# ArmastusChen/Learning-Continuous-Implicit-Representation-for-Near-Periodic-Patterns

Measured on AMD Instinct MI355X. Metric: fitted pixels/sec/GPU (512^2 grid, 256-wide MLP) + iters-to-target-PSNR, higher is better.
Workload: dtype bf16

## Files before the change

### learning-continuous-implicit-representation-for-near-periodic-patterns_amd/csrc/npp_api.hip

```cpp
#include <math.h>
#include <stdarg.h>
#include <stdio.h>
#include <string.h>
#include <vector>

#include "npp_common.h"
#include "npp_stash_census.h"

namespace npp {

static thread_local char g_err[512] = "";

void set_error(const char* fmt, ...) {
  va_list ap;
  va_start(ap, fmt);
  vsnprintf(g_err, sizeof(g_err), fmt, ap);
  va_end(ap);
}

int check_launch(const char* what) {
  hipError_t e = hipGetLastError();
  if (e != hipSuccess) {
    set_error("%s: %s", what, hipGetErrorString(e));
    return NPP_ERR_LAUNCH;
  }
  return NPP_OK;
}

bool smem_attr(SmemOnce& once, const void* fn, int bytes) {
  int dev = 0;
  if (hipGetDevice(&dev) != hipSuccess) return false;
  const unsigned long long bit = 1ull << (dev & 63);
  if (__atomic_load_n(&once.done, __ATOMIC_RELAXED) & bit) return true;
  if (hipFuncSetAttribute(fn, hipFuncAttributeMaxDynamicSharedMemorySize, bytes) != hipSuccess) return false;
  __atomic_fetch_or(&once.done, bit, __ATOMIC_RELAXED);
  return true;
}

static const char* kNames[kNumLayers] = {
    "periodic_linears.0", "periodic_linears.1", "periodic_linears.2", "periodic_linears.3",
    "periodic_linears.4", "periodic_linears.5", "periodic_linears.6", "periodic_linears.7",
    "feature_linear1",    "scale_linears.0",    "feature_linear2",    "pos_linears.0",
    "rgb_linear"};
static char g_name_buf[kNumLayers * 2][40];

NPP_HD float fwd_pack_value(const float* P, const NetDesc& d, int l, int ks, int nt, int lane, int j) {
  const int col = fwd_col(d.K, l, ks, lane >> 5, j);
  if (col < 0) return 0.0f;
  const int row = nt * 32 + (lane & 31);
  return P[d.w_off[l] + (int64_t)row * d.n_in[l] + col];
}
NPP_HD float bwd_pack_value(const float* P, const NetDesc& d, const BwdDesc& b, int v, int ns, int kt,
                            int lane, int j) {
  const int l = b.layer[v];
  const int n = 16 * ns + perm16(lane >> 5, j);
  const int col = b.col0[v] + kt * 32 + (lane & 31);
  return P[d.w_off[l] + (int64_t)n * d.n_in[l] + col];
}

NPP_HD bool fwd_unit(const NetDesc& d, int64_t u, int& l, int& ks, int& nt, int& lane) {
  for (l = 0; l < kNumLayers; ++l) {
    if (!d.present[l] || d.nt_f[l] == 0) continue;
    const int64_t n = (int64_t)d.ks_f[l] * d.nt_f[l] * 64;
    if (u >= d.wf_off[l] && u < d.wf_off[l] + n) {
      int64_t r = u - d.wf_off[l];
      lane = (int)(r & 63);
      r >>= 6;
      nt = (int)(r % d.nt_f[l]);
      ks = (int)(r / d.nt_f[l]);
      return true;
    }
  }
  return false;
}
NPP_HD bool bwd_unit(const BwdDesc& b, int64_t u, int& v, int& ns, int& kt, int& lane) {
  for (v = 0; v < kNumBwd; ++v) {
    if (!b.present[v]) continue;
    const int64_t n = (int64_t)b.ns[v] * kNT * 64;
    if (u >= b.off16[v] && u < b.off16[v] + n) {
      int64_t r = u - b.off16[v];
      lane = (int)(r & 63);
      r >>= 6;
      kt = (int)(r % kNT);
      ns = (int)(r / kNT);
      return true;
    }
  }
  return false;
}

__global__ void pack_weights_kernel(const float* __restrict__ P, bf16x8* __restrict__ wf,
                                    bf16x8* __restrict__ wb, NetDesc d, BwdDesc b, int64_t nf,
                                    int64_t nb) {
  const int64_t u = (int64_t)blockIdx.x * blockDim.x + threadIdx.x;
  if (u < nf) {
    int l, ks, nt, lane;
    if (fwd_unit(d, u, l, ks, nt, lane)) {
      bf16x8 r;
#pragma unroll
      for (int j = 0; j < 8; ++j) r[j] = (__bf16)fwd_pack_value(P, d, l, ks, nt, lane, j);
      wf[u] = r;
    }
  } else if (u < nf + nb) {
    const int64_t ub = u - nf;
    int v, ns, kt, lane;
    if (bwd_unit(b, ub, v, ns, kt, lane)) {
      bf16x8 r;
#pragma unroll
      for (int j = 0; j < 8; ++j) r[j] = (__bf16)bwd_pack_value(P, d, b, v, ns, kt, lane, j);
      wb[ub] = r;
    }
  }
}

struct AdamPackArgs {
  float *p, *m, *v;
  const float* g;
  int64_t n;
  int32_t n_slabs;
  int64_t slab_stride;
  float step_size, b1, b2, inv_sqrt_bc2, eps;
  AdamTail tail;
  __bf16 *wf, *wb;
  uint32_t magic[kNumLayers];
  const StackIter* iter;
  int64_t blob_stride, slab_img_stride, wf_stride, wb_stride;
  int32_t lat_stride, zero_stride;
  int64_t pl_stride;
  const float* hp;
};

__global__ __launch_bounds__(256) void adam_pack_kernel(AdamPackArgs a_in, NetDesc d_arg, BwdDesc b_arg) {
  AdamPackArgs a = a_in;
  if (a.iter) {
    const int y = (int)blockIdx.y;
    const StackIter it = a.iter[y];
    if (!it.active) return;
    a.p += y * a.blob_stride; a.m += y * a.blob_stride; a.v += y * a.blob_stride;
    a.g += y * a.slab_img_stride;
    a.wf += y * a.wf_stride; a.wb += y * a.wb_stride;
    a.step_size = it.step_size; a.inv_sqrt_bc2 = it.inv_sqrt_bc2;
    a.tail.p += y * a.lat_stride; a.tail.m += y * a.lat_stride; a.tail.v += y * a.lat_stride; a.tail.g += y * a.lat_stride;
    a.tail.zero += y * a.zero_stride;
    if (a.tail.pl_part) a.tail.pl_part += y * a.pl_stride;
    if (a.tail.loss_cur) a.tail.loss_cur += y * a.zero_stride;
  }
  if (a.hp) { a.step_size = a.hp[0]; a.inv_sqrt_bc2 = a.hp[1]; }
  __shared__ NetDesc d;
  __shared__ BwdDesc b;
  __shared__ uint32_t magic[kNumLayers];
  if (threadIdx.x == 0) {
    const uint32_t* s1 = (const uint32_t*)&d_arg;
    uint32_t* t1 = (uint32_t*)&d;
#pragma unroll
    for (int i = 0; i < (int)(sizeof(NetDesc) / 4); ++i) t1[i] = s1[i];
    const uint32_t* s2 = (const uint32_t*)&b_arg;
    uint32_t* t2 = (uint32_t*)&b;
#pragma unroll
    for (int i = 0; i < (int)(sizeof(BwdDesc) / 4); ++i) t2[i] = s2[i];
#pragma unroll
    for (int i = 0; i < kNumLayers; ++i) magic[i] = a.magic[i];
  }
  __syncthreads();
  if ((int64_t)blockIdx.x * blockDim.x * 4 >= a.n) {
    adam_tail_block(a.tail, a.step_size, a.b1, a.b2, a.inv_sqrt_bc2, a.eps);
    return;
  }
  const int64_t i = ((int64_t)blockIdx.x * blockDim.x + threadIdx.x) * 4;
  if (i >= a.n) return;
  const int cnt = (int)(a.n - i < 4 ? a.n - i : 4);
  float pn[4];
  adam_quad(a.p, a.m, a.v, a.g, i, cnt, a.n_slabs, a.slab_stride, a.step_size, a.b1, a.b2, a.inv_sqrt_bc2, a.eps, pn);
  int l = 0;
#pragma unroll
  for (int q = 1; q < kNumLayers; ++q)
    if (d.present[q] && i >= d.w_off[q]) l = q;
  int64_t r = i - d.w_off[l];
  int n = (int)__umulhi((uint32_t)r, magic[l]), k = (int)r - n * d.n_in[l];
  bool fwd4 = false;
  if (cnt == 4 && n < d.n_out[l] && (k & 3) == 0 && k + 3 < d.n_in[l]) {
    const int64_t p0 = fwd_pack_pos(d, l, n, k), p3 = fwd_pack_pos(d, l, n, k + 3);
    if (p0 >= 0 && p3 == p0 + 3 && (p0 & 3) == 0) {
      typedef __bf16 bf16x4_t __attribute__((ext_vector_type(4)));
      const bf16x4_t w4 = {(__bf16)pn[0], (__bf16)pn[1], (__bf16)pn[2], (__bf16)pn[3]};
      *(bf16x4_t*)(a.wf + p0) = w4;
      fwd4 = true;
    }
  }
#pragma unroll
  for (int e = 0; e < 4; ++e) {
    if (e < cnt) {
      if (n < d.n_out[l]) {
        const __bf16 w = (__bf16)pn[e];
        if (!fwd4) {
          const int64_t pf = fwd_pack_pos(d, l, n, k);
          if (pf >= 0) a.wf[pf] = w;
        }
        const int64_t pb = bwd_pack_pos(b, l, n, k);
        if (pb >= 0) a.wb[pb] = w;
      }
      if (++k == d.n_in[l]) { k = 0; ++n; }
      if (n >= d.n_out[l] && i + e + 1 >= d.b_off[l] + d.n_out[l]) {
        do { ++l; } while (l < kNumLayers && !d.present[l]);
        if (l >= kNumLayers) break;
        n = 0; k = 0;
      }
    }
  }
}

static uint16_t f32_to_bf16_host(float f) {
  uint32_t u;
  memcpy(&u, &f, 4);
  if ((u & 0x7fffffffu) > 0x7f800000u) return (uint16_t)((u >> 16) | 0x40);
  u += 0x7FFF + ((u >> 16) & 1);
  return (uint16_t)(u >> 16);
}

__global__ void selftest_kernel(float* out) {
  const int lane = threadIdx.x & 63;
  const int m = lane & 31, h = lane >> 5;
  bf16x8 a, b;
#pragma unroll
  for (int j = 0; j < 8; ++j) {
    const int k = 8 * h + j;
    a[j] = (__bf16)(float)(((m * 3 + k * 5) % 5) - 2);
    b[j] = (__bf16)(float)(((k * 7 + m * 2) % 4) - 1);
  }
  f32x16 acc = {};
  acc = mfma_bf16(a, b, acc);
#pragma unroll
  for (int r = 0; r < 16; ++r) out[acc_row(r, h) * 32 + m] = acc[r];
  f32x16 y = {};
#pragma unroll
  for (int s = 0; s < 2; ++s) {
    bf16x8 x = pack_acc(acc, s), a2;
#pragma unroll
    for (int j = 0; j < 8; ++j) {
      const int k = 16 * s + perm16(h, j);
      a2[j] = (__bf16)(float)(((m * 5 + k * 3) % 7) - 3);
    }
    y = mfma_bf16(a2, x, y);
  }
#pragma unroll
  for (int r = 0; r < 16; ++r) out[1024 + acc_row(r, h) * 32 + m] = y[r];

  __shared__ __attribute__((aligned(16))) char tile[16384];
  for (int u = lane; u < 1024; u += 64) {
    const int hh = u & 1, b = (u >> 1) & 31, bt = (u >> 6) & 1, ks = u >> 7;
    bf16x8 f;
#pragma unroll
    for (int j = 0; j < 8; ++j) {
      const int feat = 16 * ks + perm16(hh, j), row = bt * 32 + b;
      f[j] = (__bf16)(float)(((7 * feat + 3 * row) % 251) - 125);
    }
    *(bf16x8*)(tile + wfmt_unit(8, 0, ks, bt, b, hh)) = f;
  }
  __syncthreads();
  for (int tt = 0; tt < 4; ++tt)
    for (int t = 0; t < 4; ++t) {
      const bf16x8 f = wfrag_read(tile, wfrag_offset(tt, t, lane));
#pragma unroll
      for (int j = 0; j < 8; ++j) out[2048 + ((tt * 4 + t) * 64 + lane) * 8 + j] = (float)f[j];
    }
}

static int tune_env(const char* name, int dflt) {
  const char* e = getenv(name);
  return e && *e ? atoi(e) : dflt;
}
Tunables g_tune = {tune_env("NPP_CONV_WINK", 1), tune_env("NPP_CONV_WIN", 1), tune_env("NPP_CONV_WSTAT", 1), tune_env("NPP_CONV_PAIR", 15),
                   tune_env("NPP_LIGHT_DET", 1), tune_env("NPP_STASH8", 1)};

}

using namespace npp;

extern "C" {

int npp_version(void) { return 100; }

int npp_tune(const char* key, int value) {
  struct { const char* k; int* v; } tab[] = {{"conv_wink", &g_tune.conv_wink}, {"conv_win", &g_tune.conv_win},
                                             {"conv_wstat", &g_tune.conv_wstat}, {"conv_pair", &g_tune.conv_pair},
                                             {"stash8", &g_tune.stash8}, {"light_det", &g_tune.light_det}};
  if (key)
    for (auto& t : tab)
      if (!strcmp(key, t.k)) {
        const int old = __atomic_load_n(t.v, __ATOMIC_RELAXED);
        if (value >= 0) __atomic_store_n(t.v, value, __ATOMIC_RELAXED);
        return old;
      }
  set_error("npp_tune: unknown key '%s'", key ? key : "(null)");
  return NPP_ERR_ARG;
}
const char* npp_last_error_string(void) { return g_err; }

int npp_device_count(void) {
  int n = 0;
  hipError_t e = hipGetDeviceCount(&n);
  if (e != hipSuccess) {
    set_error("hipGetDeviceCount: %s", hipGetErrorString(e));
    (void)hipGetLastError();
    return 0;
  }
  return n;
}

static int check_kw(int K, int width) {
  if (K < 1 || K > NPP_MAX_K) { set_error("K=%d outside [1,%d]", K, NPP_MAX_K); return NPP_ERR_ARG; }
  if (width != NPP_WIDTH) {
    set_error("width=%d: this build is specialised for width %d", width, NPP_WIDTH);
    return NPP_ERR_UNSUPPORTED;
  }
  return NPP_OK;
}

int npp_param_layout(int K, int width, const char** names, int64_t* offsets, int32_t* rows,
                     int32_t* cols, int64_t* total) {
  int rc = check_kw(K, width);
  if (rc) return rc;
  const NetDesc d = make_desc(K);
  int n = 0;
  for (int l = 0; l < kNumLayers; ++l) {
    if (!d.present[l]) continue;
    for (int wb = 0; wb < 2; ++wb) {
      snprintf(g_name_buf[n], sizeof(g_name_buf[n]), "%s.%s", kNames[l], wb ? "bias" : "weight");
      if (names) names[n] = g_name_buf[n];
      if (offsets) offsets[n] = wb ? d.b_off[l] : d.w_off[l];
      if (rows) rows[n] = d.n_out[l];
      if (cols) cols[n] = wb ? 1 : d.n_in[l];
      ++n;
    }
  }
  if (total) *total = d.total_params;
  return n;
}

int64_t npp_pack_bytes(int K, int width, int which) {
  if (check_kw(K, width)) return -1;
  return 16 * (which == 0 ? make_desc(K).wf_total16 : bwd_total16(K));
}

int npp_pack_weights(const float* d_params, void* d_wf, void* d_wb, int K, int width, void* stream) {
  int rc = check_kw(K, width);
  if (rc) return rc;
  if (!d_params || !d_wf || !d_wb) { set_error("npp_pack_weights: null pointer"); return NPP_ERR_ARG; }
  const NetDesc d = make_desc(K);
  const BwdDesc b = make_bwd_desc(K);
  const int64_t nf = d.wf_total16, nb = bwd_total16(K);
  const int threads = 256;
  const int64_t blocks = (nf + nb + threads - 1) / threads;
  hipLaunchKernelGGL(pack_weights_kernel, dim3((unsigned)blocks), dim3(threads), 0, (hipStream_t)stream,
                     d_params, (bf16x8*)d_wf, (bf16x8*)d_wb, d, b, nf, nb);
  return check_launch("npp_pack_weights");
}

int npp_pack_weights_host(const float* params, void* wf, void* wb, int K, int width) {
  int rc = check_kw(K, width);
  if (rc) return rc;
  const NetDesc d = make_desc(K);
  const BwdDesc b = make_bwd_desc(K);
  uint16_t* f = (uint16_t*)wf;
  uint16_t* g = (uint16_t*)wb;
  for (int64_t u = 0; u < d.wf_total16; ++u) {
    int l, ks, nt, lane;
    if (!fwd_unit(d, u, l, ks, nt, lane)) { set_error("fwd unit %lld unmapped", (long long)u); return NPP_ERR_ARG; }
    for (int j = 0; j < 8; ++j) f[u * 8 + j] = f32_to_bf16_host(fwd_pack_value(params, d, l, ks, nt, lane, j));
  }
  const int64_t nb = bwd_total16(K);
  for (int64_t u = 0; u < nb; ++u) {
    int v, ns, kt, lane;
    if (!bwd_unit(b, u, v, ns, kt, lane)) { set_error("bwd unit %lld unmapped", (long long)u); return NPP_ERR_ARG; }
    for (int j = 0; j < 8; ++j) g[u * 8 + j] = f32_to_bf16_host(bwd_pack_value(params, d, b, v, ns, kt, lane, j));
  }
  return NPP_OK;
}

int npp_pack_scatter_host(const float* params, void* wf, void* wb, int K, int width) {
  int rc = check_kw(K, width);
  if (rc) return rc;
  const NetDesc d = make_desc(K);
  const BwdDesc b = make_bwd_desc(K);
  uint16_t* f = (uint16_t*)wf;
  uint16_t* g = (uint16_t*)wb;
  memset(f, 0, (size_t)d.wf_total16 * 16);
  memset(g, 0, (size_t)bwd_total16(K) * 16);
  for (int l = 0; l < kNumLayers; ++l) {
    if (!d.present[l]) continue;
    for (int n = 0; n < d.n_out[l]; ++n)
      for (int k = 0; k < d.n_in[l]; ++k) {
        const uint16_t w = f32_to_bf16_host(params[d.w_off[l] + (int64_t)n * d.n_in[l] + k]);
        const int64_t pf = fwd_pack_pos(d, l, n, k), pb = bwd_pack_pos(b, l, n, k);
        if (pf >= 0) {
          if (pf >= d.wf_total16 * 8) { set_error("fwd_pack_pos out of range (l=%d n=%d k=%d)", l, n, k); return NPP_ERR_ARG; }
          f[pf] = w;
        }
        if (pb >= 0) {
          if (pb >= bwd_total16(K) * 8) { set_error("bwd_pack_pos out of range (l=%d n=%d k=%d)", l, n, k); return NPP_ERR_ARG; }
          g[pb] = w;
        }
      }
  }
  return NPP_OK;
}

static int adam_pack_go(AdamPackArgs a, float* d_p, float* d_m, float* d_v, const float* d_gslabs, int64_t n, int n_slabs,
                        int64_t slab_stride, const AdamTail& tail, float beta1, float beta2, float eps, int M, int K,
                        void* d_wf, void* d_wb, void* stream, const char* who, const char* need) {
  const NetDesc d = make_desc(K);
  if (n != d.total_params || !d_p || !d_m || !d_v || !d_gslabs || !d_wf || !d_wb || n_slabs < 1 || tail.n < 0 || tail.n_zero < 0 ||
      (tail.n > 0 && (!tail.p || !tail.m || !tail.v || !tail.g)) || (tail.n_zero > 0 && !tail.zero) || slab_stride % 4 ||
      (((uintptr_t)d_p | (uintptr_t)d_m | (uintptr_t)d_v | (uintptr_t)d_gslabs) & 15)) {
    set_error("%s: bad arguments (n=%lld, expected %lld parameters; %s)", who, (long long)n, (long long)d.total_params, need);
    return NPP_ERR_ARG;
  }
  a.p = d_p; a.m = d_m; a.v = d_v; a.g = d_gslabs; a.n = n; a.n_slabs = n_slabs; a.slab_stride = slab_stride;
  a.b1 = beta1; a.b2 = beta2; a.eps = eps;
  a.tail = tail;
  a.wf = (__bf16*)d_wf; a.wb = (__bf16*)d_wb;
  for (int l = 0; l < kNumLayers; ++l) a.magic[l] = d.present[l] ? (uint32_t)((1ull << 32) / (uint64_t)d.n_in[l]) + 1u : 0u;
  const int64_t threads = (n + 3) / 4;
  hipLaunchKernelGGL(adam_pack_kernel, dim3((unsigned)((threads + 255) / 256 + 1), (unsigned)M), dim3(256), 0, (hipStream_t)stream, a, d,
                     make_bwd_desc(K));
  return check_launch(who);
}
static int adam_pack_bad(const char* who, const char* what) {
  set_error("%s: bad arguments (%s)", who, what);
  return NPP_ERR_ARG;
}
static const char* const kAdamPackNeed = "16-byte aligned blobs, slab stride % 4 == 0";

int npp_adam_step_net_pack(float* d_p, float* d_m, float* d_v, const float* d_gslabs, int64_t n, int n_slabs,
                           int64_t slab_stride, float* d_lat, float* d_lat_m, float* d_lat_v, float* d_dlat, int n_lat,
                           float* d_zero, int n_zero, float lr, float beta1, float beta2, float eps, int step, int K,
                           int width, void* d_wf, void* d_wb, float* d_pl_partials, float* d_loss_cur, void* stream) {
  int rc = check_kw(K, width);
  if (rc) return rc;
  if (step < 1) return adam_pack_bad("npp_adam_step_net_pack", "step < 1");
  const AdamWords w = adam_words(lr, beta1, beta2, step);
  AdamPackArgs a{};
  a.step_size = w.step_size; a.inv_sqrt_bc2 = w.inv_sqrt_bc2;
  return adam_pack_go(a, d_p, d_m, d_v, d_gslabs, n, n_slabs, slab_stride,
                      AdamTail{d_lat, d_lat_m, d_lat_v, d_dlat, n_lat, d_zero, n_zero, d_pl_partials, d_loss_cur}, beta1, beta2, eps,
                      1, K, d_wf, d_wb, stream, "npp_adam_step_net_pack", kAdamPackNeed);
}

int npp_adam_step_net_pack_dev(float* d_p, float* d_m, float* d_v, const float* d_gslabs, int64_t n, int n_slabs,
                               int64_t slab_stride, float* d_lat, float* d_lat_m, float* d_lat_v, float* d_dlat, int n_lat,
                               float* d_zero, int n_zero, float beta1, float beta2, float eps, const float* d_hp, int K,
                               int width, void* d_wf, void* d_wb, float* d_pl_partials, float* d_loss_cur, void* stream) {
  int rc = check_kw(K, width);
  if (rc) return rc;
  if (!d_hp || ((uintptr_t)d_hp & 3)) return adam_pack_bad("npp_adam_step_net_pack_dev", "the device words: null or not 4-byte aligned");
  AdamPackArgs a{};
  a.hp = d_hp;
  return adam_pack_go(a, d_p, d_m, d_v, d_gslabs, n, n_slabs, slab_stride,
                      AdamTail{d_lat, d_lat_m, d_lat_v, d_dlat, n_lat, d_zero, n_zero, d_pl_partials, d_loss_cur}, beta1, beta2, eps,
                      1, K, d_wf, d_wb, stream, "npp_adam_step_net_pack_dev", kAdamPackNeed);
}

int npp_adam_step_net_pack_stack(float* d_p, float* d_m, float* d_v, int64_t blob_stride, const float* d_gslabs, int64_t n,
                                 int n_slabs, int64_t slab_stride, int64_t slab_img_stride, float* d_lat, float* d_lat_m,
                                 float* d_lat_v, float* d_dlat, int n_lat, int lat_stride, float* d_zero, int n_zero,
                                 int zero_stride, float beta1, float beta2, float eps, int M, int K, int width, void* d_wf,
                                 int64_t wf_stride_bytes, void* d_wb, int64_t wb_stride_bytes, float* d_pl_partials,
                                 int64_t pl_stride, float* d_loss_cur, const void* d_iter, void* stream) {
  int rc = check_kw(K, width);
  if (rc) return rc;
  if (!d_iter || M < 1 || M > NPP_MAX_STACK || blob_stride % 4 || slab_img_stride % 4 || blob_stride < n || wf_stride_bytes % 16 ||
      wb_stride_bytes % 16)
    return adam_pack_bad("npp_adam_step_net_pack_stack", "M, the iteration records or the per-image strides");
  AdamPackArgs a{};
  a.iter = (const StackIter*)d_iter;
  a.blob_stride = blob_stride; a.slab_img_stride = slab_img_stride; a.wf_stride = wf_stride_bytes / 2; a.wb_stride = wb_stride_bytes / 2;
  a.lat_stride = lat_stride; a.zero_stride = zero_stride; a.pl_stride = pl_stride;
  return adam_pack_go(a, d_p, d_m, d_v, d_gslabs, n, n_slabs, slab_stride,
                      AdamTail{d_lat, d_lat_m, d_lat_v, d_dlat, n_lat, d_zero, n_zero, d_pl_partials, d_loss_cur}, beta1, beta2, eps,
                      M, K, d_wf, d_wb, stream, "npp_adam_step_net_pack_stack", "16-byte aligned blobs and strides");
}

int npp_train_workspace(int K, int width, int64_t Bp, int ksplit, int64_t sizes[4]) {
  int rc = check_kw(K, width);
  if (rc) return rc;
  if (Bp <= 0 || Bp % kRowTile || ksplit < 1 || !sizes) { set_error("npp_train_workspace: bad Bp/ksplit"); return NPP_ERR_ARG; }
  sizes[0] = 0;
  sizes[1] = (int64_t)act_total_ks(K) * (Bp / kRowTile) * (2048 + 1024);
  sizes[2] = (int64_t)kDzTotalKs * (Bp / kRowTile) * 2048;
  sizes[3] = (int64_t)ksplit * slab_stride_of(make_desc(K).total_params) * 4;
  return NPP_OK;
}

int64_t npp_stash8_census_words(int K, int width) {
  if (check_kw(K, width)) return -1;
  return census_words(K);
}

int npp_stash8_census_layout(int K, int width, const char** names, int32_t* formats, int32_t* features, int64_t* offsets,
                             int64_t* tile_offset) {
  int rc = check_kw(K, width);
  if (rc) return rc;
  static thread_local char name_buf[kCensusMaxArrays][12];
  const CensusDesc d = make_census_desc(K, name_buf);
  for (int i = 0; i < d.n; ++i) {
    if (names) names[i] = name_buf[i];
    if (formats) formats[i] = d.a[i].side;
    if (features) features[i] = d.a[i].features;
    if (offsets) offsets[i] = (int64_t)i * kCensusEntry;
  }
  if (tile_offset) *tile_offset = (int64_t)d.n * kCensusEntry;
  return d.n;
}

static int census_check(const char* who, const void* actF, const void* dzF, int64_t Bp, int64_t n_rows, int K, int width, const void* rec) {
  int rc = check_kw(K, width);
  if (rc) return rc;
  if (!actF || !dzF || !rec || (((uintptr_t)actF | (uintptr_t)dzF) & 15) || ((uintptr_t)rec & 7)) {
    set_error("%s: null or misaligned pointer (stash arrays 16-byte, record 8-byte aligned)", who);
    return NPP_ERR_ARG;
  }
  if (Bp <= 0 || Bp % kRowTile || Bp / kRowTile > 65536 || n_rows < 1 || n_rows > Bp) {
    set_error("%s: bad Bp=%lld (a multiple of %d, <= %d rows) / n_rows=%lld (1..Bp)", who, (long long)Bp, kRowTile, 65536 * kRowTile, (long long)n_rows);
    return NPP_ERR_ARG;
  }
  return NPP_OK;
}

int npp_stash8_census(const void* d_actF, const void* d_dzF, int64_t Bp, int64_t n_rows, int K, int width, int64_t* d_record,
                      void* stream) {
  int rc = census_check("npp_stash8_census", d_actF, d_dzF, Bp, n_rows, K, width, d_record);
  if (rc) return rc;
  CensusArgs A{};
  A.n_wg = Bp / kRowTile; A.n_rows = n_rows;
  A.act8 = (const uint8_t*)d_actF + act8_region_base(K, A.n_wg);
  A.dz8 = (const uint8_t*)d_dzF;
  A.rec = (unsigned long long*)d_record;
  A.d = make_census_desc(K);
  hipStream_t s = (hipStream_t)stream;
  const int64_t words = (int64_t)A.d.n * kCensusEntry + NPP_CENSUS_TILE_WORDS;
  hipError_t e = hipMemsetAsync(d_record, 0, (size_t)words * 8, s);
  if (e == hipSuccess) e = hipMemsetAsync(d_record + (int64_t)A.d.n * kCensusEntry + NPP_CENSUS_SCALE_MIN, 0x7f, 8, s);
  if (e != hipSuccess) { set_error("npp_stash8_census: hipMemsetAsync: %s", hipGetErrorString(e)); return NPP_ERR_LAUNCH; }
  int max_nks = 0;
  for (int i = 0; i < A.d.n; ++i) max_nks = A.d.a[i].nks > max_nks ? A.d.a[i].nks : max_nks;
  const int64_t want = ((int64_t)max_nks * A.n_wg * 64 + 4 * kCensusThreads - 1) / (4 * kCensusThreads);
  const unsigned gx = (unsigned)(want < 1 ? 1 : (want > 64 ? 64 : want));
  hipLaunchKernelGGL(stash8_census_kernel, dim3(gx, (unsigned)A.d.n + 1), dim3(kCensusThreads), 0, s, A);
  return check_launch("npp_stash8_census");
}

int npp_stash8_census_host(const void* actF, const void* dzF, int64_t Bp, int64_t n_rows, int K, int width, int64_t* record) {
  int rc = census_check("npp_stash8_census_host", actF, dzF, Bp, n_rows, K, width, record);
  if (rc) return rc;
  const int64_t n_wg = Bp / kRowTile;
  stash8_census_host((const uint8_t*)actF + act8_region_base(K, n_wg), (const uint8_t*)dzF, n_wg, n_rows, K, record);
  return NPP_OK;
}

int npp_selftest_mfma(void* d_scratch, void* stream) {
  if (!d_scratch) { set_error("npp_selftest_mfma: null scratch"); return NPP_ERR_ARG; }
  hipStream_t s = (hipStream_t)stream;
  hipLaunchKernelGGL(selftest_kernel, dim3(1), dim3(64), 0, s, (float*)d_scratch);
  int rc = check_launch("npp_selftest_mfma");
  if (rc) return rc;
  std::vector<float> out(2048 + 8192);
  hipError_t e = hipMemcpyAsync(out.data(), d_scratch, (2048 + 8192) * sizeof(float), hipMemcpyDeviceToHost, s);
  if (e == hipSuccess) e = hipStreamSynchronize(s);
  if (e != hipSuccess) { set_error("selftest copy: %s", hipGetErrorString(e)); return NPP_ERR_LAUNCH; }
  int A[32][16], B[16][32], D[32][32], A2[32][32];
  for (int m = 0; m < 32; ++m)
    for (int k = 0; k < 16; ++k) { A[m][k] = ((m * 3 + k * 5) % 5) - 2; B[k][m] = ((k * 7 + m * 2) % 4) - 1; }
  for (int m = 0; m < 32; ++m)
    for (int k = 0; k < 32; ++k) A2[m][k] = ((m * 5 + k * 3) % 7) - 3;
  for (int i = 0; i < 32; ++i)
    for (int j = 0; j < 32; ++j) {
      int acc = 0;
      for (int k = 0; k < 16; ++k) acc += A[i][k] * B[k][j];
      D[i][j] = acc;
    }
  for (int i = 0; i < 32; ++i)
    for (int j = 0; j < 32; ++j) {
      if (out[i * 32 + j] != (float)D[i][j]) {
        set_error("selftest: plain MFMA lane map mismatch at (%d,%d): got %g want %d", i, j, out[i * 32 + j], D[i][j]);
        return NPP_ERR_SELFTEST;
      }
      int acc = 0;
      for (int k = 0; k < 32; ++k) acc += A2[i][k] * D[k][j];
      if (out[1024 + i * 32 + j] != (float)acc) {
        set_error("selftest: accumulator-as-operand chain mismatch at (%d,%d): got %g want %d", i, j,
                  out[1024 + i * 32 + j], acc);
        return NPP_ERR_SELFTEST;
      }
    }
  for (int tt = 0; tt < 4; ++tt)
    for (int t = 0; t < 4; ++t)
      for (int lane = 0; lane < 64; ++lane)
        for (int j = 0; j < 8; ++j) {
          const int feat = 32 * tt + (lane & 31), row = 16 * t + 8 * (lane >> 5) + j;
          const float want = (float)(((7 * feat + 3 * row) % 251) - 125);
          const float got = out[2048 + ((tt * 4 + t) * 64 + lane) * 8 + j];
          if (got != want) {
            set_error("selftest: W-format transposed read mismatch tt=%d t=%d lane=%d j=%d: got %g want %g", tt, t, lane, j, got, want);
            return NPP_ERR_SELFTEST;
          }
        }
  return NPP_OK;
}

}
```

Measured before the change: 46.99 million.

## Tile Adam pack kernel into 4x4 weight tiles with shuffle-transposed backward stores

Adam parameter updates for aligned weight layers are now assigned per 4x4 tile, with a host-side region table mapping blocks to layers. Each thread updates four contiguous weights, writes them vectorized to the forward pack, and exchanges values with three lanes via xor-shuffles so that it can store a transposed 4-wide vector into the backward pack. Previously those backward writes were scattered scalar stores. The shared descriptor copy is spread across all threads, and tail blocks exit before it. The cost is a larger kernel argument and more index math per thread.

New measurement: 46.84 million. No clear change (-0.3%).

```diff
diff --git a/learning-continuous-implicit-representation-for-near-periodic-patterns_amd/csrc/npp_api.hip b/learning-continuous-implicit-representation-for-near-periodic-patterns_amd/csrc/npp_api.hip
--- a/learning-continuous-implicit-representation-for-near-periodic-patterns_amd/csrc/npp_api.hip
+++ b/learning-continuous-implicit-representation-for-near-periodic-patterns_amd/csrc/npp_api.hip
@@ -111,6 +111,45 @@
       wb[ub] = r;
     }
   }
+}
+
+#ifndef NPP_ADAM_THREADS
+#define NPP_ADAM_THREADS 256
+#endif
+constexpr int kAdamThreads = NPP_ADAM_THREADS;
+constexpr int kMaxAdamRegions = 2 * kNumLayers + 2;
+struct AdamRegion {
+  int64_t off, end;
+  int32_t block0;
+  int32_t layer;
+  int32_t tiles_per_row, ntiles;
+};
+struct AdamRegions {
+  int32_t n, n_blocks;
+  AdamRegion reg[kMaxAdamRegions];
+};
+static AdamRegions adam_regions(const NetDesc& d) {
+  AdamRegions R{};
+  int block = 0;
+  int64_t gen0 = 0;
+  auto close_generic = [&](int64_t end) {
+    if (end <= gen0) return;
+    AdamRegion& r = R.reg[R.n++];
+    r.off = gen0; r.end = end; r.block0 = block; r.layer = -1;
+    block += (int)(((end - gen0 + 3) / 4 + kAdamThreads - 1) / kAdamThreads);
+  };
+  for (int l = 0; l < kNumLayers; ++l) {
+    if (!d.present[l] || d.nt_f[l] == 0 || d.n_in[l] % 4 || d.n_out[l] % 4 || d.w_off[l] % 4) continue;
+    close_generic(d.w_off[l]);
+    AdamRegion& r = R.reg[R.n++];
+    r.off = d.w_off[l]; r.end = d.w_off[l] + (int64_t)d.n_out[l] * d.n_in[l]; r.block0 = block; r.layer = l;
+    r.tiles_per_row = d.n_in[l] / 4; r.ntiles = (d.n_out[l] / 4) * r.tiles_per_row;
+    block += (4 * r.ntiles + kAdamThreads - 1) / kAdamThreads;
+    gen0 = r.end;
+  }
+  close_generic(d.total_params);
+  R.n_blocks = block;
+  return R;
 }
 
 struct AdamPackArgs {
@@ -130,7 +169,7 @@
   const float* hp;
 };
 
-__global__ __launch_bounds__(256) void adam_pack_kernel(AdamPackArgs a_in, NetDesc d_arg, BwdDesc b_arg) {
+__global__ __launch_bounds__(kAdamThreads) void adam_pack_kernel(AdamPackArgs a_in, NetDesc d_arg, BwdDesc b_arg, AdamRegions rg) {
   AdamPackArgs a = a_in;
   if (a.iter) {
     const int y = (int)blockIdx.y;
@@ -146,31 +185,74 @@
     if (a.tail.loss_cur) a.tail.loss_cur += y * a.zero_stride;
   }
   if (a.hp) { a.step_size = a.hp[0]; a.inv_sqrt_bc2 = a.hp[1]; }
+  const int bx = (int)blockIdx.x, tid = (int)threadIdx.x;
+  if (bx >= rg.n_blocks) {
+    adam_tail_block(a.tail, a.step_size, a.b1, a.b2, a.inv_sqrt_bc2, a.eps);
+    return;
+  }
   __shared__ NetDesc d;
   __shared__ BwdDesc b;
   __shared__ uint32_t magic[kNumLayers];
-  if (threadIdx.x == 0) {
-    const uint32_t* s1 = (const uint32_t*)&d_arg;
-    uint32_t* t1 = (uint32_t*)&d;
-#pragma unroll
-    for (int i = 0; i < (int)(sizeof(NetDesc) / 4); ++i) t1[i] = s1[i];
-    const uint32_t* s2 = (const uint32_t*)&b_arg;
-    uint32_t* t2 = (uint32_t*)&b;
-#pragma unroll
-    for (int i = 0; i < (int)(sizeof(BwdDesc) / 4); ++i) t2[i] = s2[i];
-#pragma unroll
-    for (int i = 0; i < kNumLayers; ++i) magic[i] = a.magic[i];
-  }
+  {
+    constexpr int n1 = (int)(sizeof(NetDesc) / 4), n2 = (int)(sizeof(BwdDesc) / 4);
+    static_assert(sizeof(NetDesc) % 4 == 0 && sizeof(BwdDesc) % 4 == 0, "dword copies");
+    for (int i = tid; i < n1 + n2 + kNumLayers; i += kAdamThreads) {
+      if (i < n1) ((uint32_t*)&d)[i] = ((const uint32_t*)&d_arg)[i];
+      else if (i < n1 + n2) ((uint32_t*)&b)[i - n1] = ((const uint32_t*)&b_arg)[i - n1];
+      else magic[i - n1 - n2] = a_in.magic[i - n1 - n2];
+    }
+  }
+  AdamRegion R = rg.reg[0];
+#pragma unroll
+  for (int j = 1; j < kMaxAdamRegions; ++j)
+    if (j < rg.n && bx >= rg.reg[j].block0) R = rg.reg[j];
+  const int u = (bx - R.block0) * kAdamThreads + tid;
+  typedef __bf16 bf16x4_t __attribute__((ext_vector_type(4)));
+
+  if (R.layer >= 0) {
+    const bool active = u < 4 * R.ntiles;
+    const int t = u >> 2, r = u & 3;
+    const int g4 = t / R.tiles_per_row, n0 = 4 * g4, k = 4 * (t - g4 * R.tiles_per_row), n_in = 4 * R.tiles_per_row;
+    float pn[4];
+    if (active)
+      adam_quad(a.p, a.m, a.v, a.g, R.off + (int64_t)(n0 + r) * n_in + k, 4, a.n_slabs, a.slab_stride, a.step_size, a.b1, a.b2,
+                a.inv_sqrt_bc2, a.eps, pn);
+    __syncthreads();
+    if (!active) return;
+    const int l = R.layer;
+    uint32_t x[4], y[4];
+#pragma unroll
+    for (int e = 0; e < 4; ++e) y[e] = x[e] = (uint32_t)__builtin_bit_cast(uint16_t, (__bf16)pn[e]);
+    const int64_t p0 = fwd_pack_pos(d, l, n0 + r, k), p3 = fwd_pack_pos(d, l, n0 + r, k + 3);
+    if (p0 >= 0 && p3 == p0 + 3 && (p0 & 3) == 0) {
+      *(uint2*)(a.wf + p0) = make_uint2(x[0] | (x[1] << 16), x[2] | (x[3] << 16));
+    } else {
+#pragma unroll
+      for (int e = 0; e < 4; ++e) {
+        const int64_t pf = fwd_pack_pos(d, l, n0 + r, k + e);
+        if (pf >= 0) a.wf[pf] = (__bf16)pn[e];
+      }
+    }
+#pragma unroll
+    for (int sft = 1; sft < 4; ++sft) {
+      const int pr = r ^ sft;
+      const uint32_t send = pr == 0 ? x[0] : pr == 1 ? x[1] : pr == 2 ? x[2] : x[3];
+      const uint32_t got = (uint32_t)__shfl_xor((int)send, sft, 64);
+#pragma unroll
+      for (int e = 0; e < 4; ++e) y[e] = e == pr ? got : y[e];
+    }
+    const int64_t q0 = bwd_pack_pos(b, l, n0, k + r);
+    if (q0 >= 0) *(uint2*)(a.wb + q0) = make_uint2(y[0] | (y[1] << 16), y[2] | (y[3] << 16));
+    return;
+  }
+
+  const int64_t i = R.off + (int64_t)u * 4;
+  const bool active = i < R.end;
+  const int cnt = (int)(R.end - i < 4 ? R.end - i : 4);
+  float pn[4];
+  if (active) adam_quad(a.p, a.m, a.v, a.g, i, cnt, a.n_slabs, a.slab_stride, a.step_size, a.b1, a.b2, a.inv_sqrt_bc2, a.eps, pn);
   __syncthreads();
-  if ((int64_t)blockIdx.x * blockDim.x * 4 >= a.n) {
-    adam_tail_block(a.tail, a.step_size, a.b1, a.b2, a.inv_sqrt_bc2, a.eps);
-    return;
-  }
-  const int64_t i = ((int64_t)blockIdx.x * blockDim.x + threadIdx.x) * 4;
-  if (i >= a.n) return;
-  const int cnt = (int)(a.n - i < 4 ? a.n - i : 4);
-  float pn[4];
-  adam_quad(a.p, a.m, a.v, a.g, i, cnt, a.n_slabs, a.slab_stride, a.step_size, a.b1, a.b2, a.inv_sqrt_bc2, a.eps, pn);
+  if (!active) return;
   int l = 0;
 #pragma unroll
   for (int q = 1; q < kNumLayers; ++q)
@@ -181,7 +263,6 @@
   if (cnt == 4 && n < d.n_out[l] && (k & 3) == 0 && k + 3 < d.n_in[l]) {
     const int64_t p0 = fwd_pack_pos(d, l, n, k), p3 = fwd_pack_pos(d, l, n, k + 3);
     if (p0 >= 0 && p3 == p0 + 3 && (p0 & 3) == 0) {
-      typedef __bf16 bf16x4_t __attribute__((ext_vector_type(4)));
       const bf16x4_t w4 = {(__bf16)pn[0], (__bf16)pn[1], (__bf16)pn[2], (__bf16)pn[3]};
       *(bf16x4_t*)(a.wf + p0) = w4;
       fwd4 = true;
@@ -420,9 +501,9 @@
   a.tail = tail;
   a.wf = (__bf16*)d_wf; a.wb = (__bf16*)d_wb;
   for (int l = 0; l < kNumLayers; ++l) a.magic[l] = d.present[l] ? (uint32_t)((1ull << 32) / (uint64_t)d.n_in[l]) + 1u : 0u;
-  const int64_t threads = (n + 3) / 4;
-  hipLaunchKernelGGL(adam_pack_kernel, dim3((unsigned)((threads + 255) / 256 + 1), (unsigned)M), dim3(256), 0, (hipStream_t)stream, a, d,
-                     make_bwd_desc(K));
+  const AdamRegions rg = adam_regions(d);
+  hipLaunchKernelGGL(adam_pack_kernel, dim3((unsigned)(rg.n_blocks + 1), (unsigned)M), dim3(kAdamThreads), 0, (hipStream_t)stream, a, d,
+                     make_bwd_desc(K), rg);
   return check_launch(who);
 }
 static int adam_pack_bad(const char* who, const char* what) {
```
